# resibots/limbo

Measured on AMD Instinct MI355X. Metric: GP compute()+log_lik evaluations/sec at N=4096 D=6 fp64, higher is better.
Workload: dtype f64

## Files before the change

### limbo_amd/csrc/dev.h

```cpp
#pragma once
#include <hip/hip_runtime.h>
#include <hip/hip_ext.h>
#include <stdint.h>

#define GPE_MAX_THETA 64
#define GPE_MAX_P 8

struct KParams {
    int kind;
    int D;
    int Din;
    int k_lam;
    double sf2;
    double inv_l;
    double diag_add;
    double noise;
    double inv_ell[GPE_MAX_THETA];
};

typedef double d4_t __attribute__((ext_vector_type(4)));

static __device__ __forceinline__ d4_t mfma_f64(double a, double b, d4_t c)
{
    return __builtin_amdgcn_mfma_f64_16x16x4f64(a, b, c, 0, 0, 0);
// ... 117 lines not shown
    double A[GPE_MAX_THETA];
};
void launch_lambda_rows(hipStream_t s, double* Xt, int64_t ld, int64_t col0, int64_t n, const LamParams& lp);

void launch_diag(hipStream_t s, double* A, int64_t lda, int jb, double* Xt, int* info, int64_t goff, int half_form);
typedef unsigned long long gpe_epoch_t;
void launch_panel_step(hipStream_t s, double* A, int64_t lda, int64_t j0, int64_t M, int nt, const double* Xt_cur,
                       double* Xt_next, int do_next, int* info, double* Hs, int64_t dnext, int64_t dfirst, int dinit,
                       double* Dacc, gpe_epoch_t* hflag);
void launch_panel256(hipStream_t s, double* A, int64_t lda, int64_t p0, int64_t M, double* Xt, int* info, int64_t dnext,
                     double* Dacc, double* S22, double* S22_next, hipEvent_t stop = nullptr);
#define GPE_TAIL_MAX 8192
void flow_gate_enter(hipStream_t s);
void flow_gate_leave(hipStream_t s);
void flow_gate_forget(hipStream_t s);
struct FlowGate {
    hipStream_t s;
    bool on;
    explicit FlowGate(hipStream_t s_, bool engage = true) : s(s_), on(engage)
    {
        if (on)
            flow_gate_enter(s);
    }
    ~FlowGate()
    {
        if (on)
            flow_gate_leave(s);
    }
    FlowGate(const FlowGate&) = delete;
    FlowGate& operator=(const FlowGate&) = delete;
};
int debug_tail_order(int nt, int nb, int lag, int pair);
void debug_chain_split(int wave, int* units10, int* cols);
static inline int64_t tail_tiles(int64_t nt, int64_t nb) { return nt * nb - nt * (nt - 1) / 2; }
static inline int64_t tail_buf_doubles(int64_t nt, int64_t nb) { return nt * 3072 + tail_tiles(nt, nb) * 4096; }
struct TailGen {
    const double* Xg;
    int64_t ldx, Ns;
    const double* Om;
    int64_t ldom;
    double* Al;
    int64_t ldal;
    int P;
    const KParams* kp;
};
int ragged_split(int64_t k, int64_t scratch_doubles, int* kc_out);
bool launch_ragged_finish(hipStream_t s, double* C, int64_t ldc, const double* A, int64_t ld, int64_t jb, int64_t P, int64_t k,
                          double* scratch, int64_t scratch_doubles, double* Xt, int* info, int64_t goff);
bool launch_ragged_update(hipStream_t s, double* C, int64_t ldc, const double* A, int64_t ld, int64_t m, int64_t n, int64_t k,
                          double* scratch, int64_t scratch_doubles);
void launch_tail(hipStream_t s, double* A, int64_t lda, int64_t t0, int64_t t1, int64_t N64, int64_t M, double* Xt_all, int* info,
                 double* buf_cur, double* buf_next, const TailGen* gen = nullptr);
#define GPE_S22_TILE 20
#define GPE_S22_TILES 9
#define GPE_HEAD_TILES 66
void launch_head_copy(hipStream_t s, double* A, int64_t lda, int64_t p0, int nt0, int nf, const double* H);
void launch_diag_inv(hipStream_t s, const double* L, int64_t ldl, int64_t N, int64_t b0, int64_t nblocks,
                     double* Xt_all);

struct GemmArgs {
    double* C; int64_t ldc;
    const double* A; int64_t lda; int a_kmajor;
    const double* B; int64_t ldb; int b_kmajor;
    int64_t m, n, k;
    int tri; int64_t grow0, gcol0;
    int ktri;
// ... 149 lines not shown
```

### limbo_amd/csrc/engine.hip

```cpp
#include "../../include/gpe.h"
#include "../../include/gpe_joint.h"
#include "dev.h"

#include <algorithm>
#include <cmath>
#include <cstdio>
#include <cstdlib>
#include <cstring>
#include <iterator>
#include <atomic>
#include <chrono>
#include <map>
#include <dlfcn.h>
#include <fcntl.h>
#include <sys/file.h>
#include <sys/stat.h>
#include <thread>
#include <unistd.h>
#include <mutex>
#include <string>
#include <vector>

thread_local BatchLaunch g_batch;

namespace {
struct TraceRec {
    const char* name;
    hipStream_t stream;
    hipEvent_t e0, e1;
    unsigned gx, gy, gz, bx;
    bool own_stop;
};
std::mutex g_trace_mu;
std::vector<TraceRec> g_trace;
// ... 1525 lines not shown
    std::lock_guard<std::mutex> lk(g_trace_mu);
    for (auto& r : g_trace) {
        g_trace_pool.push_back(r.e0);
        g_trace_pool.push_back(r.e1);
    }
    g_trace.clear();
    g_trace_state.store(on ? 1 : 0);
    return GPE_OK;
}
int gpe_trace_dump(const char* path)
{
    if (!path)
        return GPE_ERR_ARG;
    hipDeviceSynchronize();
    std::lock_guard<std::mutex> lk(g_trace_mu);
    FILE* f = fopen(path, "w");
    if (!f)
        return GPE_ERR_ARG;
    std::map<hipStream_t, int> sid;
    hipEvent_t ref = g_trace.empty() ? nullptr : g_trace[0].e0;
    for (auto& r : g_trace) {
        float a = 0.f, b = 0.f;
        if (hipEventElapsedTime(&a, ref, r.e0) != hipSuccess || hipEventElapsedTime(&b, ref, r.e1) != hipSuccess)
            continue;
        if (!sid.count(r.stream))
            sid[r.stream] = (int)sid.size();
        fprintf(f, "%10.2f %10.2f %d %s grid=%u,%u,%u block=%u\n", 1e3 * a, 1e3 * b, sid[r.stream], r.name, r.gx, r.gy, r.gz, r.bx);
    }
    fclose(f);
    return GPE_OK;
}

int gpe_debug_tail_order(int nt, int nb, int lag, int pair) { return debug_tail_order(nt, nb, lag, pair); }
int gpe_debug_ragged_split(int64_t k, int64_t scratch_doubles, int* kc)
{
    if (!kc)
        return -1;
    *kc = 0;
    return ragged_split(k, scratch_doubles, kc);
}
int gpe_debug_tri_tile_map(int64_t m, int64_t n, int64_t grow0, int64_t gcol0, int* out, int cap)
{
    if (m <= 0 || n <= 0 || !out || cap <= 0 || (m + 127) / 128 >= 65536 || (n + 127) / 128 >= 32768)
        return -1;
    return debug_tri_tile_map(m, n, grow0, gcol0, out, cap);
}
int gpe_debug_chain_split(int wave, int* units10, int* cols)
{
    if (wave < 0 || wave > 7 || !units10 || !cols)
        return -1;
    debug_chain_split(wave, units10, cols);
    return 0;
}
int gpe_debug_inv_plan(int64_t n, int64_t ld, int nbins, int load_pct, int64_t* out, int64_t cap_rows)
{
    return inv2_debug_plan(n, ld, nbins, load_pct, out, cap_rows);
}

int gpe_debug_tail_plan(int64_t n, int p, int g, int64_t tail_max, int64_t tall_max, int64_t batch_tail_max, int64_t* out8)
{
    if (!out8 || n < 1 || p < 1)
        return GPE_ERR_ARG;
    debug_tail_plan(n, p, g, tail_max, tall_max, batch_tail_max, out8);
    return GPE_OK;
}

// ... 18 lines not shown
```

### limbo_amd/csrc/potrf.hip

```cpp
#include "dev.h"
#include <hip/hip_ext.h>
#include <atomic>
#include <cstdio>

#define NB 64
#ifndef DIAG_ABL
#define DIAG_ABL 0
#endif
#ifdef DIAG_TIMING
__device__ long long g_diag_arr[16][8];
__device__ long long g_diag_ts[32];
#ifdef DIAG_NO_STAMPS
#define ARR(G, w) do { } while (0)
#define TS(i) do { } while (0)
#else
#define ARR(G, w) do { if ((threadIdx.x & 63) == 0 && blockIdx.x == 0) g_diag_arr[G][w] = clock64(); } while (0)
#define TS(i) do { if (threadIdx.x == 0) g_diag_ts[i] = clock64(); } while (0)
#endif
#else
#define TS(i) do { } while (0)
#define ARR(G, w) do { } while (0)
#endif
#ifdef DIAG_TIMING
__device__ long long g_panel_ts[64];
// ... 388 lines not shown
        GPE_LAUNCH(k_diag_full, dim3(1, 1, g_batch.G), dim3(256), 0, s, A, lda, jb, Xt, info, goff, g_batch.bt);
}

#define PS 80

template <bool BKM, int KLEN, int RBN, int BS = XS>
static __device__ __forceinline__ void mmk(const double* __restrict__ Aop, int ak0, const double* __restrict__ Bop,
                                           int bk0, int wm, int wn, int lane, double (&acc)[2][RBN])
{
    const int ar = wm + (lane & 15), bc = wn + (lane & 3), kq = lane >> 4;
#pragma unroll
    for (int ks = 0; ks < KLEN; ks += 4) {
        double af[2], bf[RBN];
#pragma unroll
        for (int x = 0; x < 2; ++x)
            af[x] = Aop[(ak0 + ks + kq) * PS + ar + 16 * x];
#pragma unroll
        for (int x = 0; x < RBN; ++x)
            bf[x] = BKM ? Bop[(bc + 4 * x) * BS + bk0 + ks + kq] : Bop[(bk0 + ks + kq) * PS + bc + 4 * x];
#pragma unroll
        for (int n = 0; n < RBN; ++n)
#pragma unroll
            for (int m = 0; m < 2; ++m)
                acc[m][n] = mfma4(af[m], bf[n], acc[m][n]);
    }
}
template <bool BKM>
static __device__ __forceinline__ void mm64(const double* __restrict__ Aop, const double* __restrict__ Bop, int wm, int wn,
                                            int lane, double (&acc)[2][4])
{
    mmk<BKM, NB, 4>(Aop, 0, Bop, 0, wm, wn, lane, acc);
}

static __device__ __forceinline__ void trsm_tile_full(double* __restrict__ T, const double* __restrict__ Bx, int lane, int wave)
{
    const int wm = (wave & 1) * 32, wn = (wave >> 1) * 16;
    const int drow = 4 * ((lane >> 2) & 3) + (lane >> 4), dcol = lane & 3;
    double y[2][4];
#pragma unroll
    for (int m = 0; m < 2; ++m)
#pragma unroll
        for (int n = 0; n < 4; ++n)
            y[m][n] = 0.0;
    switch (wave >> 1) {
    case 0: mmk<true, 16, 4>(T, 0, Bx, 0, wm, wn, lane, y); break;
    case 1: mmk<true, 32, 4>(T, 0, Bx, 0, wm, wn, lane, y); break;
    case 2: mmk<true, 48, 4>(T, 0, Bx, 0, wm, wn, lane, y); break;
    default: mmk<true, 64, 4>(T, 0, Bx, 0, wm, wn, lane, y); break;
    }
    __syncthreads();
#pragma unroll
    for (int m = 0; m < 2; ++m)
#pragma unroll
        for (int n = 0; n < 4; ++n)
            T[(wn + 4 * n + dcol) * PS + wm + 16 * m + drow] = y[m][n];
    __syncthreads();
}

struct TileRegs {
    double v[8];
    __device__ __forceinline__ void load(const double* __restrict__ G, int64_t ld, int nrows)
    {
        const int i = threadIdx.x & 63, kk0 = threadIdx.x >> 6;
        const int ic = i < nrows ? i : nrows - 1;
#pragma unroll
        for (int q = 0; q < 8; ++q)
// ... 333 lines not shown
            b[q] = __hip_atomic_load(g + 8 * q * NB, __ATOMIC_RELAXED, POLL_FIRST_SCOPE);
    }
    __device__ __forceinline__ void finish(const double* G, int spin_limit, int* __restrict__ info)
    {
        const unsigned long long SENT = ~0ull;
        const unsigned long long* g = reinterpret_cast<const unsigned long long*>(G) + (threadIdx.x & 63) + (threadIdx.x >> 6) * NB;
        int spins = 0;
        while (b[0] == SENT || b[1] == SENT || b[2] == SENT || b[3] == SENT || b[4] == SENT || b[5] == SENT || b[6] == SENT
               || b[7] == SENT) {
            if (++spins > spin_limit) {
                info[2] = 1;
                break;
            }
            poll_one(G + NB * NB - 1, spin_limit, info);
            if (b[0] == SENT) b[0] = __hip_atomic_load(g + 0 * NB, __ATOMIC_RELAXED, __HIP_MEMORY_SCOPE_AGENT);
            if (b[1] == SENT) b[1] = __hip_atomic_load(g + 8 * NB, __ATOMIC_RELAXED, __HIP_MEMORY_SCOPE_AGENT);
            if (b[2] == SENT) b[2] = __hip_atomic_load(g + 16 * NB, __ATOMIC_RELAXED, __HIP_MEMORY_SCOPE_AGENT);
            if (b[3] == SENT) b[3] = __hip_atomic_load(g + 24 * NB, __ATOMIC_RELAXED, __HIP_MEMORY_SCOPE_AGENT);
            if (b[4] == SENT) b[4] = __hip_atomic_load(g + 32 * NB, __ATOMIC_RELAXED, __HIP_MEMORY_SCOPE_AGENT);
            if (b[5] == SENT) b[5] = __hip_atomic_load(g + 40 * NB, __ATOMIC_RELAXED, __HIP_MEMORY_SCOPE_AGENT);
            if (b[6] == SENT) b[6] = __hip_atomic_load(g + 48 * NB, __ATOMIC_RELAXED, __HIP_MEMORY_SCOPE_AGENT);
            if (b[7] == SENT) b[7] = __hip_atomic_load(g + 56 * NB, __ATOMIC_RELAXED, __HIP_MEMORY_SCOPE_AGENT);
        }
    }
    __device__ __forceinline__ void store(double* __restrict__ T) const
    {
        const int i = threadIdx.x & 63, kk0 = threadIdx.x >> 6;
#pragma unroll
        for (int q = 0; q < 8; ++q)
            T[(kk0 + 8 * q) * PS + i] = __longlong_as_double((long long)b[q]);
    }
};

template <int S, bool PUBHALF>
static __device__ __forceinline__ void p256_half_solve(const P256& x, double* __restrict__ T, double* __restrict__ Ld,
                                                       const double (&own)[8], double (&a2)[2][4], const bool acc_on,
                                                       const double* __restrict__ Sq, double* __restrict__ pub)
{
    const int lane = threadIdx.x & 63, wave = __builtin_amdgcn_readfirstlane(threadIdx.x >> 6);
    const int wm = (wave & 1) * 32, wn = (wave >> 1) * 16;
    const int hn = (wave >> 1) * 8;
    const int crow = wm + (lane & 31), ccol = wn + (lane >> 5);
    const int drow = 4 * ((lane >> 2) & 3) + (lane >> 4), dcol = lane & 3;
    double* Bx = x.Bx;
    P2TS(6 * S + 0);
#pragma unroll
    for (int it = 0; it < 8; ++it)
        T[(ccol + 2 * it) * PS + crow] = own[it];
    const unsigned long long SENT = ~0ull;
    const unsigned long long* Sp = reinterpret_cast<const unsigned long long*>(Sq) + threadIdx.x;
    {
        unsigned long long b[4];
#pragma unroll
        for (int q = 0; q < 4; ++q)
            b[q] = __hip_atomic_load(Sp + 512 * q, __ATOMIC_RELAXED, POLL_FIRST_SCOPE);
        int spins = 0;
        while (b[0] == SENT || b[1] == SENT || b[2] == SENT || b[3] == SENT) {
            if (++spins > x.spin_limit) {
                x.info[2] = 1;
                break;
            }
            poll_one(Sq + 1023, x.spin_limit, x.info);
            poll_one(Sq + 1024 + 32 * 31, x.spin_limit, x.info);
#pragma unroll
            for (int q = 0; q < 4; ++q)
                if (b[q] == SENT)
// ... 330 lines not shown
    static const bool fault = getenv("GPE_HANDOVER_FAULT") && atoi(getenv("GPE_HANDOVER_FAULT")) != 0;
    const int spin_limit = fault ? -16 : GPE_FLOW_SPIN_LIMIT;
    const int64_t rows = M - (p0 + NB);
    if (rows <= 0)
        return;
    const dim3 grid((unsigned)((rows + NB - 1) / NB)), block(512);
    FlowGate gate(s);
    if (stop)
        GPE_LAUNCH_STOP("k_panel256", k_panel256, grid, block, 0, s, stop, A, lda, p0, M, Xt, info, dnext, Dacc, spin_limit, S22, S22_next);
    else
        GPE_LAUNCH(k_panel256, grid, block, 0, s, A, lda, p0, M, Xt, info, dnext, Dacc, spin_limit, S22, S22_next);
}

struct TailArgs {
    double* A;
    int64_t lda, t0;
    int nt, nb;
    int nfull;
    int rhs_rows;
    double* Xt;
    int* info;
    double *LP, *SP, *LPn, *SPn;
    int spin_limit;
    const int* order;
    const double* Xg;
    int64_t ldx, Ns;
    const double* Om;
    int64_t ldom;
    double* Al;
    int64_t ldal;
    int P;
};
#define TAIL_LDS_DOUBLES (4 * NB * PS)
static_assert(TAIL_LDS_DOUBLES >= NB * XS + 3 * NB * PS && TAIL_LDS_DOUBLES * 8 <= 160 * 1024, "k_tail LDS carve");
static __device__ __forceinline__ int tail_tile_id(int nb, int b, int c) { return c * nb - (c * (c - 1)) / 2 + (b - c); }

static __device__ __forceinline__ void tail_gen_tile(const TailArgs& a, const KParams* __restrict__ kp, int64_t I, int64_t J0,
                                                     double (&out)[8])
{
    if (I >= a.Ns) {
        const double* om = a.Om + (I - a.Ns) * a.ldom;
#pragma unroll
        for (int it = 0; it < 8; ++it)
            out[it] = om[J0 + 2 * it];
        return;
    }
    double z[8];
#pragma unroll
    for (int it = 0; it < 8; ++it)
        z[it] = 0.0;
    const int D = kp->D;
    for (int d = 0; d < D; ++d) {
        const double* xr = a.Xg + (int64_t)d * a.ldx;
        const double xi = xr[I], ie = kp->inv_ell[d];
#pragma unroll
        for (int it = 0; it < 8; ++it) {
            const double q = (xi - xr[J0 + 2 * it]) * ie;
            z[it] = fma(q, q, z[it]);
        }
    }
    const int kind = kp->kind;
    const double sf2 = kp->sf2, da = kp->diag_add;
#pragma unroll
    for (int it = 0; it < 8; ++it)
        out[it] = kfun_fast_rt(kind, z[it], sf2) + (I == J0 + 2 * it ? da : 0.0);
}

// ... 301 lines not shown
        X22[(e0 >> 5) * 34 + (e0 & 31)] = __longlong_as_double((long long)xc[0]);
        X22[(e1 >> 5) * 34 + (e1 & 31)] = __longlong_as_double((long long)xc[1]);
    }
    __syncthreads();
    TTS2(x, true, 3);
    double y2[2][2] = {{0.0, 0.0}, {0.0, 0.0}};
    tri_solve32(T, 32, X22, wm, hn, lane, y2);
#pragma unroll
    for (int m = 0; m < 2; ++m)
#pragma unroll
        for (int n = 0; n < 2; ++n)
            Ys[(hn + 4 * n + dcol) * PS + wm + 16 * m + drow] = y2[m][n];
    __syncthreads();
    TTS2(x, true, 4);
    syrk40<32>(Ys, 0, wave, lane, a2v);
    syrk40_store_neg(Dl, wave, lane, a2v);
    {
        const int i = threadIdx.x & 63, kk0 = threadIdx.x >> 6;
#pragma unroll
        for (int q = 0; q < 4; ++q) {
            const int col = kk0 + 8 * q;
            __hip_atomic_store(pub + i + NB * (32 + col), Ys[col * PS + i], __ATOMIC_RELAXED, __HIP_MEMORY_SCOPE_AGENT);
        }
    }
#pragma unroll
    for (int m = 0; m < 2; ++m)
#pragma unroll
        for (int n = 0; n < 2; ++n)
            T[(32 + hn + 4 * n + dcol) * PS + wm + 16 * m + drow] = y2[m][n];
    TTS2(x, true, 5);
}

static __device__ __forceinline__ void tail_tile_solve(const P256& x, double* __restrict__ lds, const double (&own)[8],
                                                       const double* __restrict__ Sq, double* __restrict__ pub, const bool near)
{
    const int lane = threadIdx.x & 63, wave = __builtin_amdgcn_readfirstlane(threadIdx.x >> 6);
    const int wm = (wave & 1) * 32, wn = (wave >> 1) * 16;
    const int hn = tri_solve_cols(wave);
    const int crow = wm + (lane & 31), ccol = wn + (lane >> 5);
    const int drow = 4 * ((lane >> 2) & 3) + (lane >> 4), dcol = lane & 3;
    double* const T = lds + CH_T;
    double* const X11 = lds + CH_X11;
    double* const Ld = lds + CH_LD;
    double* const Ys = lds + CH_YS;
    double* const X22 = lds + CH_X22;
    const unsigned long long SENT = ~0ull;
    const unsigned long long* Sp = reinterpret_cast<const unsigned long long*>(Sq) + threadIdx.x;
#pragma unroll
    for (int it = 0; it < 8; ++it)
        T[(ccol + 2 * it) * PS + crow] = own[it];
    {
        unsigned long long xb[4];
#pragma unroll
        for (int q = 0; q < 4; ++q)
            xb[q] = __hip_atomic_load(Sp + 512 * q, __ATOMIC_RELAXED, POLL_FIRST_SCOPE);
        if (near)
            chain_watch<4>(Sp, xb, x.spin_limit, x.info);
        else {
            int spins = 0;
            while (xb[0] == SENT || xb[1] == SENT || xb[2] == SENT || xb[3] == SENT) {
                if (++spins > x.spin_limit) {
                    x.info[2] = 1;
                    break;
                }
                poll_one(Sq + 1023, x.spin_limit, x.info);
                poll_one(Sq + 1024 + 32 * 31, x.spin_limit, x.info);
#pragma unroll
                for (int q = 0; q < 4; ++q)
                    if (xb[q] == SENT)
                        xb[q] = __hip_atomic_load(Sp + 512 * q, __ATOMIC_RELAXED, __HIP_MEMORY_SCOPE_AGENT);
            }
        }
#pragma unroll
        for (int q = 0; q < 2; ++q) {
            const int e = threadIdx.x + 512 * q;
            X11[(e >> 5) * 34 + (e & 31)] = __longlong_as_double((long long)xb[q]);
            Ld[(e & 31) * 34 + (e >> 5)] = __longlong_as_double((long long)xb[2 + q]);
        }
    }
    __syncthreads();
    double y1[2][2] = {{0.0, 0.0}, {0.0, 0.0}};
    tri_solve32(T, 0, X11, wm, hn, lane, y1);
#pragma unroll
    for (int m = 0; m < 2; ++m)
#pragma unroll
        for (int n = 0; n < 2; ++n)
            Ys[(hn + 4 * n + dcol) * PS + wm + 16 * m + drow] = y1[m][n];
    __syncthreads();
    double u[2][2] = {{0.0, 0.0}, {0.0, 0.0}};
    mmk<true, 32, 2, 34>(Ys, 0, Ld, 0, wm, hn, lane, u);
#pragma unroll
    for (int m = 0; m < 2; ++m)
#pragma unroll
        for (int n = 0; n < 2; ++n) {
            double* t = T + (32 + hn + 4 * n + dcol) * PS + wm + 16 * m + drow;
            *t = *t - u[m][n];
            T[(hn + 4 * n + dcol) * PS + wm + 16 * m + drow] = y1[m][n];
        }
    {
        const int i = threadIdx.x & 63, kk0 = threadIdx.x >> 6;
#pragma unroll
        for (int q = 0; q < 4; ++q) {
            const int col = kk0 + 8 * q;
            __hip_atomic_store(pub + i + NB * col, Ys[col * PS + i], __ATOMIC_RELAXED, __HIP_MEMORY_SCOPE_AGENT);
        }
    }
    {
        unsigned long long xc[2];
        xc[0] = __hip_atomic_load(Sp + 2048, __ATOMIC_RELAXED, POLL_FIRST_SCOPE);
        xc[1] = __hip_atomic_load(Sp + 2048 + 512, __ATOMIC_RELAXED, POLL_FIRST_SCOPE);
        if (near)
            chain_watch<2>(Sp + 2048, xc, x.spin_limit, x.info);
        else {
            int spins = 0;
            while (xc[0] == SENT || xc[1] == SENT) {
                if (++spins > x.spin_limit) {
                    x.info[2] = 1;
                    break;
                }
                poll_one(Sq + 2048 + 1023, x.spin_limit, x.info);
                if (xc[0] == SENT)
                    xc[0] = __hip_atomic_load(Sp + 2048, __ATOMIC_RELAXED, __HIP_MEMORY_SCOPE_AGENT);
                if (xc[1] == SENT)
                    xc[1] = __hip_atomic_load(Sp + 2048 + 512, __ATOMIC_RELAXED, __HIP_MEMORY_SCOPE_AGENT);
            }
        }
        const int e0 = threadIdx.x, e1 = threadIdx.x + 512;
        X22[(e0 >> 5) * 34 + (e0 & 31)] = __longlong_as_double((long long)xc[0]);
        X22[(e1 >> 5) * 34 + (e1 & 31)] = __longlong_as_double((long long)xc[1]);
    }
    __syncthreads();
    double y2[2][2] = {{0.0, 0.0}, {0.0, 0.0}};
    tri_solve32(T, 32, X22, wm, hn, lane, y2);
#pragma unroll
    for (int m = 0; m < 2; ++m)
#pragma unroll
        for (int n = 0; n < 2; ++n)
            Ys[(hn + 4 * n + dcol) * PS + wm + 16 * m + drow] = y2[m][n];
    __syncthreads();
    {
        const int i = threadIdx.x & 63, kk0 = threadIdx.x >> 6;
#pragma unroll
        for (int q = 0; q < 4; ++q) {
            const int col = kk0 + 8 * q;
            __hip_atomic_store(pub + i + NB * (32 + col), Ys[col * PS + i], __ATOMIC_RELAXED, __HIP_MEMORY_SCOPE_AGENT);
        }
    }
#pragma unroll
    for (int m = 0; m < 2; ++m)
#pragma unroll
        for (int n = 0; n < 2; ++n)
            T[(32 + hn + 4 * n + dcol) * PS + wm + 16 * m + drow] = y2[m][n];
    __syncthreads();
}

static __device__ __forceinline__ void tail_body(const TailArgs& a, const int wgid, double* __restrict__ lds,
                                                 const KParams* __restrict__ kp = nullptr)
{
    const int lane = threadIdx.x & 63, wave = __builtin_amdgcn_readfirstlane(threadIdx.x >> 6);
    const int wm = (wave & 1) * 32, wn = (wave >> 1) * 16;
    const int crow = wm + (lane & 31), ccol = wn + (lane >> 5);
    int c = 0, b;
    if (a.order) {
        b = __builtin_amdgcn_readfirstlane(a.order[2 * wgid]);
        c = __builtin_amdgcn_readfirstlane(a.order[2 * wgid + 1]);
    }
    else {
        int id = wgid, colh = a.nb;
        while (id >= colh) {
            id -= colh;
            ++c;
            --colh;
        }
        b = c + id;
    }
    const int slot = tail_tile_id(a.nb, b, c);
    const bool mute = a.spin_limit < 0;
    P256 x;
    x.A = a.A;
    x.lda = a.lda;
    x.p0 = a.t0;
    x.R0 = a.t0 + (int64_t)NB * b;
    x.Xt = a.Xt;
    x.info = a.info;
    x.mute = mute;
    x.spin_limit = mute ? -a.spin_limit : a.spin_limit;
    x.nrows = b < a.nfull ? NB : a.rhs_rows;
    x.want_d = false;
    x.Bx = lds;
    x.T0 = lds + NB * XS;
    x.T1 = x.T0 + NB * PS;
    x.T2 = x.T1 + NB * PS;
    x.S22 = a.SP;
    x.HP = a.LP;
    double* const myslot = a.LP + (int64_t)slot * (NB * NB);
    {
        unsigned long long* nx = reinterpret_cast<unsigned long long*>(a.LPn + (int64_t)slot * (NB * NB));
#pragma unroll
        for (int q = 0; q < 8; ++q)
            nx[threadIdx.x + 512 * q] = ~0ull;
        if (b == c) {
            unsigned long long* ns = reinterpret_cast<unsigned long long*>(a.SPn + (int64_t)c * 3072);
#pragma unroll
            for (int q = 0; q < 6; ++q)
                ns[threadIdx.x + 512 * q] = ~0ull;
        }
    }
    if (b == c + 1 && b < a.nt)
        return;
    const int crc = crow < x.nrows ? crow : x.nrows - 1;
    double cv[8];
    if (kp) {
        tail_gen_tile(a, kp, x.R0 + crc, a.t0 + (int64_t)NB * c + ccol, cv);
        if (a.Al && b >= a.nfull && threadIdx.x < NB)
            for (int p = 0; p < a.P; ++p)
                reinterpret_cast<unsigned long long*>(a.Al)[a.t0 + (int64_t)NB * c + threadIdx.x + (int64_t)p * a.ldal] = ~0ull;
    }
    else {
#pragma unroll
        for (int it = 0; it < 8; ++it)
            cv[it] = a.A[x.R0 + crc + (a.t0 + (int64_t)NB * c + ccol + 2 * it) * a.lda];
    }
    if (b == c) {
        double* const Dl = lds + CH_D;
        double* const Ltb = lds + CH_AUX;
        double* const invd = Ltb + DIAG_LTB;
        DiagSync* const sy = reinterpret_cast<DiagSync*>(invd + NB);
        if (c > 0) {
            double cl[8];
            if (kp)
                tail_gen_tile(a, kp, x.R0 + crow, a.t0 + (int64_t)NB * (c - 1) + ccol, cl);
            else {
#pragma unroll
                for (int it = 0; it < 8; ++it)
                    cl[it] = a.A[x.R0 + crow + (a.t0 + (int64_t)NB * (c - 1) + ccol + 2 * it) * a.lda];
            }
            tail_chain_updates_and_crossing(a, x, lds, c, cl, cv);
            TTS(c, 1);
        }
        else {
#pragma unroll
            for (int it = 0; it < 8; ++it)
                Dl[crow * XS + ccol + 2 * it] = cv[it];
            diag_flow_init(sy);
        }
        __syncthreads();
        DiagEarly ea;
        ea.mute = mute;
        ea.S = a.SP + (int64_t)c * 3072;
        TTS(c, 2);
        diag_flow(Dl, Ltb, invd, sy, a.A + x.R0 + x.R0 * a.lda, a.lda, a.Xt + (int64_t)c * (NB * NB), a.info, x.R0, wave, lane,
                  invd + NB + 8, &ea);
        TTS(c, 3);
        if (c > 0) {
            __syncthreads();
            const int i = threadIdx.x & 63, kk0 = threadIdx.x >> 6;
            double* Ag = a.A + x.R0 + (a.t0 + (int64_t)NB * (c - 1)) * a.lda;
            const double* T = lds + CH_T;
#pragma unroll
            for (int q = 0; q < 8; ++q) {
                const int col = kk0 + 8 * q;
                Ag[i + (int64_t)col * a.lda] = T[col * PS + i];
            }
        }
        return;
    }
    PolledTile pa, pb;
    if (c > 0) {
        pa.issue(a.LP + (int64_t)tail_tile_id(a.nb, b, 0) * (NB * NB));
        pb.issue(a.LP + (int64_t)tail_tile_id(a.nb, c, 0) * (NB * NB));
    }
    double a2[2][4] = {{0.0, 0.0, 0.0, 0.0}, {0.0, 0.0, 0.0, 0.0}};
#pragma unroll 1
    for (int s = 0; s < c; ++s) {
        double* const opA = lds + (s & 1) * (2 * NB * PS);
        double* const opB = opA + NB * PS;
        pa.finish(a.LP + (int64_t)tail_tile_id(a.nb, b, s) * (NB * NB), x.spin_limit, x.info);
        pa.store(opA);
        pb.finish(a.LP + (int64_t)tail_tile_id(a.nb, c, s) * (NB * NB), x.spin_limit, x.info);
        pb.store(opB);
        if (s + 1 < c) {
            pa.issue(a.LP + (int64_t)tail_tile_id(a.nb, b, s + 1) * (NB * NB));
            pb.issue(a.LP + (int64_t)tail_tile_id(a.nb, c, s + 1) * (NB * NB));
        }
        __syncthreads();
        mm64<false>(opA, opB, wm, wn, lane, a2);
    }
    if (c > 0) {
        double a2r[8];
        wave_tile_to_rows(a2, a2r, lane);
#pragma unroll
        for (int it = 0; it < 8; ++it)
            cv[it] -= a2r[it];
        __syncthreads();
    }
    tail_tile_solve(x, lds, cv, a.SP + (int64_t)c * 3072, myslot, b - c <= 3);
    {
// ... 264 lines not shown
        const int me = pos[tid(t.b, t.c)];
        if (t.b == t.c) {
            int last = -1;
            for (int s2 = 0; s2 < t.c - 1; ++s2)
                last = std::max(last, std::max(owner(t.c, s2), owner(t.c - 1, s2)));
            if (last > me) {
                if (dlead <= 0)
                    legal = false;
                ++blocked[(size_t)me + 1];
                --blocked[(size_t)last + 1];
            }
            if (t.c > 0)
                legal = legal && dpos(t.c - 1) < me;
        }
        else if (!(t.b == t.c + 1 && t.b < nt)) {
            for (int s2 = 0; s2 < t.c && legal; ++s2)
                legal = owner(t.b, s2) < me && owner(t.c, s2) < me;
            legal = legal && dpos(t.c) < me;
        }
        if (!legal)
            break;
    }
    for (size_t q = 1, run = 0; q < blocked.size() && legal; ++q) {
        run += blocked[q];
        legal = (int)run <= TAIL_DLEAD_MAX_BLOCKED;
    }
    flat.assign(2 * ts.size(), 0);
    for (size_t i = 0; i < ts.size(); ++i) {
        flat[2 * i] = ts[i].b;
        flat[2 * i + 1] = ts[i].c;
    }
    return legal;
}
static const int* tail_order(int nt, int nb, int dlead, int lag)
{
    const int W = 0;
    if (dlead <= 0 && lag <= 0)
        return nullptr;
    static std::mutex mu;
    static std::map<std::array<int, 6>, int*> cache;
    int dev = 0;
    (void)hipGetDevice(&dev);
    const std::array<int, 6> key{dev, nt, nb, dlead, lag, 0};
    std::lock_guard<std::mutex> lk(mu);
    auto it = cache.find(key);
    if (it != cache.end())
        return it->second;
    std::vector<int> flat;
    int* d = nullptr;
    if (build_tail_order(nt, nb, W, lag, flat, dlead) || (dlead > 0 && build_tail_order(nt, nb, W, lag, flat, 0))) {
        if (hipMalloc(&d, sizeof(int) * flat.size()) != hipSuccess || hipMemcpy(d, flat.data(), sizeof(int) * flat.size(), hipMemcpyHostToDevice) != hipSuccess)
            d = nullptr;
    }
    else
        fprintf(stderr, "gpe: tail_order(%d, %d, lead %d, lag %d) violates a dependency — column-by-column order used\n", nt, nb, dlead, lag);
    cache[key] = d;
    return d;
}
void debug_chain_split(int wave, int* units10, int* cols)
{
    for (int q = 0; q < 5; ++q)
        syrk40_units(wave, q, units10[2 * q], units10[2 * q + 1]);
    *cols = tri_solve_cols(wave);
}
int debug_tail_order(int nt, int nb, int lag, int pair)
{
    if (pair)
        return -1;
    if (nt < 1 || nb < nt || nb > 4096)
        return -1;
    std::vector<int> flat;
    if (!build_tail_order(nt, nb, 0, lag, flat, 0))
        return 0;
    if (!build_tail_order(nt, nb, 0, lag, flat, TAIL_DLEAD))
        return 0;
    std::vector<char> seen((size_t)nt * nb, 0);
    size_t n = 0;
    for (size_t i = 0; i + 1 < flat.size(); i += 2) {
        const int b = flat[i], c = flat[i + 1];
        if (c < 0 || c >= nt || b < c || b >= nb || seen[(size_t)c * nb + b])
            return 0;
        seen[(size_t)c * nb + b] = 1;
        ++n;
    }
    return n == (size_t)(nt * nb - nt * (nt - 1) / 2) ? 1 : 0;
}

void launch_tail(hipStream_t s, double* A, int64_t lda, int64_t t0, int64_t t1, int64_t N64, int64_t M, double* Xt_all, int* info,
                 double* buf_cur, double* buf_next, const TailGen* gen)
{
    TailArgs a{};
    a.A = A;
    a.lda = lda;
    a.t0 = t0;
    a.nt = (int)((t1 - t0) / NB);
    a.nfull = (int)((N64 - t0) / NB);
    a.rhs_rows = (int)(M - N64);
    a.nb = a.nfull + (a.rhs_rows > 0 ? 1 : 0);
    a.Xt = Xt_all + (t0 / NB) * (NB * NB);
    a.info = info;
    a.SP = buf_cur;
    a.LP = buf_cur + (int64_t)a.nt * 3072;
    a.SPn = buf_next;
    a.LPn = buf_next + (int64_t)a.nt * 3072;
    static const bool fault = getenv("GPE_HANDOVER_FAULT") && atoi(getenv("GPE_HANDOVER_FAULT")) != 0;
    a.spin_limit = fault ? -16 : GPE_FLOW_SPIN_LIMIT;
    static const int ord_lag = getenv("GPE_TAIL_LAG") ? atoi(getenv("GPE_TAIL_LAG")) : 3;
    a.order = tail_order(a.nt, a.nb, g_batch.bt ? 0 : TAIL_DLEAD, ord_lag);
    const int64_t tiles = tail_tiles(a.nt, a.nb);
    if (gen) {
        a.Xg = gen->Xg;
        a.ldx = gen->ldx;
        a.Ns = gen->Ns;
        a.Om = gen->Om;
        a.ldom = gen->ldom;
        a.Al = gen->Al;
        a.ldal = gen->ldal;
        a.P = gen->P;
    }
    FlowGate gate(s);
    if (g_batch.bt)
        GPE_LAUNCH(k_tail_b, dim3((unsigned)(tiles * g_batch.G)), dim3(512), 0, s, a, g_batch.bt);
    else if (gen)
        GPE_LAUNCH(k_tail_g, dim3((unsigned)tiles), dim3(512), 0, s, a, *gen->kp);
    else
        GPE_LAUNCH(k_tail, dim3((unsigned)tiles), dim3(512), 0, s, a);
}

__global__ __launch_bounds__(512) void k_upd_fused(GemmArgs g, double* __restrict__ A, int64_t lda, int64_t p0, int64_t pe,
                                                   double* __restrict__ Xt_next, int* __restrict__ info,
                                                   const double* __restrict__ Dacc)
{
    constexpr int GEMM_LDS = 4 * Glds64Shape<16>::STAGE, DIAG_LDS = 2 * NB * PS;
    constexpr int LDS_DOUBLES = GEMM_LDS > DIAG_LDS ? GEMM_LDS : DIAG_LDS;
    __shared__ __attribute__((aligned(16))) double lds[LDS_DOUBLES];
    if (blockIdx.x + 1 < gridDim.x) {
        gemm_glds64_body<16, 4, 8>(g, lds, (int)blockIdx.x, (int)gridDim.x - 1, true);
        return;
    }
    static_assert(NB * XS + DIAG_LTB + NB + 8 + DIAG_XW_DOUBLES <= 2 * NB * PS,
                  "[Ls | Ltb | invd | sync | Xw] is carved out of the two operand tiles");
    double* T0 = lds;
// ... 214 lines not shown
```

Measured before the change: 939.5.

## Pair vertically adjacent tail tiles in one workgroup to share B operand loads

Adds a 'duo' mode to the Cholesky tail kernel. One workgroup now updates and solves two vertically adjacent off-diagonal tiles of the same column, reusing the shared B-panel and the triangular factor fetch across both. A new dependency-checked ordering builder emits paired entries flagged by a high bit, and the launch grid shrinks to the number of entries. This cuts global polling and loads and the workgroup count, at the cost of longer per-workgroup critical paths, more LDS use and less parallelism in the dependency-driven schedule.

```diff
diff --git a/include/gpe_tail_duo.h b/include/gpe_tail_duo.h
--- /dev/null
+++ b/include/gpe_tail_duo.h
@@ -0,0 +1,17 @@
+#ifndef GPE_TAIL_DUO_H
+#define GPE_TAIL_DUO_H
+
+#include "gpe.h"
+
+#ifdef __cplusplus
+extern "C" {
+#endif
+
+#define GPE_TAIL_DUO_BIT 0x40000000
+
+int gpe_debug_tail_duo_order(int nt, int nb, int nfull, int lag, int strict, int* out, int cap);
+
+#ifdef __cplusplus
+}
+#endif
+#endif
diff --git a/limbo_amd/csrc/dev.h b/limbo_amd/csrc/dev.h
--- a/limbo_amd/csrc/dev.h
+++ b/limbo_amd/csrc/dev.h
@@ -173,6 +173,7 @@
 };
 int debug_tail_order(int nt, int nb, int lag, int pair);
 void debug_chain_split(int wave, int* units10, int* cols);
+int debug_tail_duo_order(int nt, int nb, int nfull, int lag, int strict, int* out, int cap);
 static inline int64_t tail_tiles(int64_t nt, int64_t nb) { return nt * nb - nt * (nt - 1) / 2; }
 static inline int64_t tail_buf_doubles(int64_t nt, int64_t nb) { return nt * 3072 + tail_tiles(nt, nb) * 4096; }
 struct TailGen {
diff --git a/limbo_amd/csrc/engine.hip b/limbo_amd/csrc/engine.hip
--- a/limbo_amd/csrc/engine.hip
+++ b/limbo_amd/csrc/engine.hip
@@ -1,5 +1,6 @@
 #include "../../include/gpe.h"
 #include "../../include/gpe_joint.h"
+#include "../../include/gpe_tail_duo.h"
 #include "dev.h"
 
 #include <algorithm>
@@ -1591,6 +1592,10 @@
 }
 
 int gpe_debug_tail_order(int nt, int nb, int lag, int pair) { return debug_tail_order(nt, nb, lag, pair); }
+int gpe_debug_tail_duo_order(int nt, int nb, int nfull, int lag, int strict, int* out, int cap)
+{
+    return debug_tail_duo_order(nt, nb, nfull, lag, strict, out, cap);
+}
 int gpe_debug_ragged_split(int64_t k, int64_t scratch_doubles, int* kc)
 {
     if (!kc)
diff --git a/limbo_amd/csrc/potrf.hip b/limbo_amd/csrc/potrf.hip
--- a/limbo_amd/csrc/potrf.hip
+++ b/limbo_amd/csrc/potrf.hip
@@ -444,6 +444,32 @@
     mmk<BKM, NB, 4>(Aop, 0, Bop, 0, wm, wn, lane, acc);
 }
 
+template <int KLEN>
+static __device__ __forceinline__ void mmk2(const double* __restrict__ A0, const double* __restrict__ A1, const double* __restrict__ Bop,
+                                            int wm, int wn, int lane, double (&acc0)[2][4], double (&acc1)[2][4])
+{
+    const int ar = wm + (lane & 15), bc = wn + (lane & 3), kq = lane >> 4;
+#pragma unroll
+    for (int ks = 0; ks < KLEN; ks += 4) {
+        double af0[2], af1[2], bf[4];
+#pragma unroll
+        for (int x = 0; x < 2; ++x) {
+            af0[x] = A0[(ks + kq) * PS + ar + 16 * x];
+            af1[x] = A1[(ks + kq) * PS + ar + 16 * x];
+        }
+#pragma unroll
+        for (int x = 0; x < 4; ++x)
+            bf[x] = Bop[(ks + kq) * PS + bc + 4 * x];
+#pragma unroll
+        for (int n = 0; n < 4; ++n)
+#pragma unroll
+            for (int m = 0; m < 2; ++m) {
+                acc0[m][n] = mfma4(af0[m], bf[n], acc0[m][n]);
+                acc1[m][n] = mfma4(af1[m], bf[n], acc1[m][n]);
+            }
+    }
+}
+
 static __device__ __forceinline__ void trsm_tile_full(double* __restrict__ T, const double* __restrict__ Bx, int lane, int wave)
 {
     const int wm = (wave & 1) * 32, wn = (wave >> 1) * 16;
@@ -843,6 +869,41 @@
     }
 };
 
+struct PolledHalf {
+    unsigned long long b[4];
+    __device__ __forceinline__ void issue(const double* G, int H)
+    {
+        const unsigned long long* g = reinterpret_cast<const unsigned long long*>(G) + (threadIdx.x & 63) + ((threadIdx.x >> 6) + 32 * H) * NB;
+#pragma unroll
+        for (int q = 0; q < 4; ++q)
+            b[q] = __hip_atomic_load(g + 8 * q * NB, __ATOMIC_RELAXED, POLL_FIRST_SCOPE);
+    }
+    __device__ __forceinline__ void finish(const double* G, int H, int spin_limit, int* __restrict__ info)
+    {
+        const unsigned long long SENT = ~0ull;
+        const unsigned long long* g = reinterpret_cast<const unsigned long long*>(G) + (threadIdx.x & 63) + ((threadIdx.x >> 6) + 32 * H) * NB;
+        int spins = 0;
+        while (b[0] == SENT || b[1] == SENT || b[2] == SENT || b[3] == SENT) {
+            if (++spins > spin_limit) {
+                info[2] = 1;
+                break;
+            }
+            poll_one(G + 32 * NB * (H + 1) - 1, spin_limit, info);
+            if (b[0] == SENT) b[0] = __hip_atomic_load(g + 0 * NB, __ATOMIC_RELAXED, __HIP_MEMORY_SCOPE_AGENT);
+            if (b[1] == SENT) b[1] = __hip_atomic_load(g + 8 * NB, __ATOMIC_RELAXED, __HIP_MEMORY_SCOPE_AGENT);
+            if (b[2] == SENT) b[2] = __hip_atomic_load(g + 16 * NB, __ATOMIC_RELAXED, __HIP_MEMORY_SCOPE_AGENT);
+            if (b[3] == SENT) b[3] = __hip_atomic_load(g + 24 * NB, __ATOMIC_RELAXED, __HIP_MEMORY_SCOPE_AGENT);
+        }
+    }
+    __device__ __forceinline__ void store(double* __restrict__ T) const
+    {
+        const int i = threadIdx.x & 63, kk0 = threadIdx.x >> 6;
+#pragma unroll
+        for (int q = 0; q < 4; ++q)
+            T[(kk0 + 8 * q) * PS + i] = __longlong_as_double((long long)b[q]);
+    }
+};
+
 template <int S, bool PUBHALF>
 static __device__ __forceinline__ void p256_half_solve(const P256& x, double* __restrict__ T, double* __restrict__ Ld,
                                                        const double (&own)[8], double (&a2)[2][4], const bool acc_on,
@@ -1239,7 +1300,9 @@
     int P;
 };
 #define TAIL_LDS_DOUBLES (4 * NB * PS)
+#define TAIL_DUO_BIT (1 << 30)
 static_assert(TAIL_LDS_DOUBLES >= NB * XS + 3 * NB * PS && TAIL_LDS_DOUBLES * 8 <= 160 * 1024, "k_tail LDS carve");
+static_assert(6 * 32 * PS <= TAIL_LDS_DOUBLES, "k_tail LDS carve of a pair workgroup: two sets of three k-half operands");
 static __device__ __forceinline__ int tail_tile_id(int nb, int b, int c) { return c * nb - (c * (c - 1)) / 2 + (b - c); }
 
 static __device__ __forceinline__ void tail_gen_tile(const TailArgs& a, const KParams* __restrict__ kp, int64_t I, int64_t J0,
@@ -1607,7 +1670,8 @@
 }
 
 static __device__ __forceinline__ void tail_tile_solve(const P256& x, double* __restrict__ lds, const double (&own)[8],
-                                                       const double* __restrict__ Sq, double* __restrict__ pub, const bool near)
+                                                       const double* __restrict__ Sq, double* __restrict__ pub, const bool near,
+                                                       const bool fetch = true)
 {
     const int lane = threadIdx.x & 63, wave = __builtin_amdgcn_readfirstlane(threadIdx.x >> 6);
     const int wm = (wave & 1) * 32, wn = (wave >> 1) * 16;
@@ -1624,7 +1688,7 @@
 #pragma unroll
     for (int it = 0; it < 8; ++it)
         T[(ccol + 2 * it) * PS + crow] = own[it];
-    {
+    if (fetch) {
         unsigned long long xb[4];
 #pragma unroll
         for (int q = 0; q < 4; ++q)
@@ -1680,7 +1744,7 @@
             __hip_atomic_store(pub + i + NB * col, Ys[col * PS + i], __ATOMIC_RELAXED, __HIP_MEMORY_SCOPE_AGENT);
         }
     }
-    {
+    if (fetch) {
         unsigned long long xc[2];
         xc[0] = __hip_atomic_load(Sp + 2048, __ATOMIC_RELAXED, POLL_FIRST_SCOPE);
         xc[1] = __hip_atomic_load(Sp + 2048 + 512, __ATOMIC_RELAXED, POLL_FIRST_SCOPE);
@@ -1729,6 +1793,96 @@
     __syncthreads();
 }
 
+static __device__ __forceinline__ void tail_pair(const TailArgs& a, const P256& x, double* __restrict__ lds, const int b, const int c,
+                                                 double (&cv)[8], double* __restrict__ myslot, const KParams* __restrict__ kp)
+{
+    const int lane = threadIdx.x & 63, wave = __builtin_amdgcn_readfirstlane(threadIdx.x >> 6);
+    const int wm = (wave & 1) * 32, wn = (wave >> 1) * 16;
+    const int crow = wm + (lane & 31), ccol = wn + (lane >> 5);
+    P256 x1 = x;
+    x1.R0 = x.R0 + NB;
+    double cu[8];
+    if (kp)
+        tail_gen_tile(a, kp, x1.R0 + crow, a.t0 + (int64_t)NB * c + ccol, cu);
+    else {
+#pragma unroll
+        for (int it = 0; it < 8; ++it)
+            cu[it] = a.A[x1.R0 + crow + (a.t0 + (int64_t)NB * c + ccol + 2 * it) * a.lda];
+    }
+    if (c > 0) {
+        PolledHalf pa, pu, pb;
+        {
+            const double* Ga = a.LP + (int64_t)tail_tile_id(a.nb, b, 0) * (NB * NB);
+            pa.issue(Ga, 0);
+            pu.issue(Ga + NB * NB, 0);
+            pb.issue(a.LP + (int64_t)tail_tile_id(a.nb, c, 0) * (NB * NB), 0);
+        }
+        double a2[2][4] = {{0.0, 0.0, 0.0, 0.0}, {0.0, 0.0, 0.0, 0.0}};
+        double a3[2][4] = {{0.0, 0.0, 0.0, 0.0}, {0.0, 0.0, 0.0, 0.0}};
+#pragma unroll 1
+        for (int s = 0; s < c; ++s) {
+            const double* Ga = a.LP + (int64_t)tail_tile_id(a.nb, b, s) * (NB * NB);
+            const double* Gb = a.LP + (int64_t)tail_tile_id(a.nb, c, s) * (NB * NB);
+#pragma unroll
+            for (int H = 0; H < 2; ++H) {
+                double* const opA = lds + H * (3 * 32 * PS);
+                double* const opU = opA + 32 * PS;
+                double* const opB = opU + 32 * PS;
+                pa.finish(Ga, H, x.spin_limit, x.info);
+                pa.store(opA);
+                pu.finish(Ga + NB * NB, H, x.spin_limit, x.info);
+                pu.store(opU);
+                pb.finish(Gb, H, x.spin_limit, x.info);
+                pb.store(opB);
+                if (H == 0) {
+                    pa.issue(Ga, 1);
+                    pu.issue(Ga + NB * NB, 1);
+                    pb.issue(Gb, 1);
+                }
+                else if (s + 1 < c) {
+                    const double* Gn = a.LP + (int64_t)tail_tile_id(a.nb, b, s + 1) * (NB * NB);
+                    pa.issue(Gn, 0);
+                    pu.issue(Gn + NB * NB, 0);
+                    pb.issue(a.LP + (int64_t)tail_tile_id(a.nb, c, s + 1) * (NB * NB), 0);
+                }
+                __syncthreads();
+                mmk2<32>(opA, opU, opB, wm, wn, lane, a2, a3);
+            }
+        }
+        double r[8];
+        wave_tile_to_rows(a2, r, lane);
+#pragma unroll
+        for (int it = 0; it < 8; ++it)
+            cv[it] -= r[it];
+        wave_tile_to_rows(a3, r, lane);
+#pragma unroll
+        for (int it = 0; it < 8; ++it)
+            cu[it] -= r[it];
+        __syncthreads();
+    }
+    const int i = threadIdx.x & 63, kk0 = threadIdx.x >> 6;
+    const double* T = lds + CH_T;
+    tail_tile_solve(x, lds, cv, a.SP + (int64_t)c * 3072, myslot, false);
+    {
+        double* Ag = a.A + x.R0 + (a.t0 + (int64_t)NB * c) * a.lda;
+#pragma unroll
+        for (int q = 0; q < 8; ++q) {
+            const int col = kk0 + 8 * q;
+            Ag[i + (int64_t)col * a.lda] = T[col * PS + i];
+        }
+    }
+    __syncthreads();
+    tail_tile_solve(x1, lds, cu, a.SP + (int64_t)c * 3072, myslot + NB * NB, false, false);
+    {
+        double* Ag = a.A + x1.R0 + (a.t0 + (int64_t)NB * c) * a.lda;
+#pragma unroll
+        for (int q = 0; q < 8; ++q) {
+            const int col = kk0 + 8 * q;
+            Ag[i + (int64_t)col * a.lda] = T[col * PS + i];
+        }
+    }
+}
+
 static __device__ __forceinline__ void tail_body(const TailArgs& a, const int wgid, double* __restrict__ lds,
                                                  const KParams* __restrict__ kp = nullptr)
 {
@@ -1736,9 +1890,12 @@
     const int wm = (wave & 1) * 32, wn = (wave >> 1) * 16;
     const int crow = wm + (lane & 31), ccol = wn + (lane >> 5);
     int c = 0, b;
+    bool duo = false;
     if (a.order) {
         b = __builtin_amdgcn_readfirstlane(a.order[2 * wgid]);
         c = __builtin_amdgcn_readfirstlane(a.order[2 * wgid + 1]);
+        duo = (b & TAIL_DUO_BIT) != 0;
+        b &= ~TAIL_DUO_BIT;
     }
     else {
         int id = wgid, colh = a.nb;
@@ -1774,6 +1931,11 @@
 #pragma unroll
         for (int q = 0; q < 8; ++q)
             nx[threadIdx.x + 512 * q] = ~0ull;
+        if (duo) {
+#pragma unroll
+            for (int q = 8; q < 16; ++q)
+                nx[threadIdx.x + 512 * q] = ~0ull;
+        }
         if (b == c) {
             unsigned long long* ns = reinterpret_cast<unsigned long long*>(a.SPn + (int64_t)c * 3072);
 #pragma unroll
@@ -1838,6 +2000,10 @@
                 Ag[i + (int64_t)col * a.lda] = T[col * PS + i];
             }
         }
+        return;
+    }
+    if (duo) {
+        tail_pair(a, x, lds, b, c, cv, myslot, kp);
         return;
     }
     PolledTile pa, pb;
@@ -2168,30 +2334,142 @@
     }
     return legal;
 }
-static const int* tail_order(int nt, int nb, int dlead, int lag)
+static bool build_tail_duo_order(int nt, int nb, int nfull, int lag, std::vector<int>& flat, int dlead)
+{
+    struct T {
+        int key, c, b, duo;
+    };
+    std::vector<T> ts;
+    for (int c = 0; c < nt; ++c)
+        for (int b = c; b < nb; ++b) {
+            int k;
+            if (b == c)
+                k = 2 * c - 3 - 2 * dlead;
+            else if (b >= nt)
+                k = 2 * (c + std::max(lag, 0));
+            else if (b == c + 1)
+                k = 2 * c;
+            else
+                k = 2 * c;
+            const bool duo = b - c >= 4 && b + 1 < nfull && b + 1 < nb && ((b + 1 < nt) || (b >= nt));
+            ts.push_back(T{k, c, b, duo ? 1 : 0});
+            if (duo)
+                ++b;
+        }
+    std::stable_sort(ts.begin(), ts.end(), [](const T& x, const T& y) {
+        if (x.key != y.key)
+            return x.key < y.key;
+        if (x.c != y.c)
+            return x.c < y.c;
+        return x.b < y.b;
+    });
+    auto tid = [&](int b, int c) { return c * nb - (c * (c - 1)) / 2 + (b - c); };
+    std::vector<int> pos((size_t)(nt * nb - nt * (nt - 1) / 2), -1);
+    for (size_t i = 0; i < ts.size(); ++i) {
+        pos[tid(ts[i].b, ts[i].c)] = (int)i;
+        if (ts[i].duo)
+            pos[tid(ts[i].b + 1, ts[i].c)] = (int)i;
+    }
+    auto dpos = [&](int c) { return pos[tid(c, c)]; };
+    auto owner = [&](int b, int s) { return (b == s + 1 && b < nt) ? dpos(b) : pos[tid(b, s)]; };
+    bool legal = true;
+    for (int p : pos)
+        legal = legal && p >= 0;
+    std::vector<int> blocked(ts.size() + 1, 0);
+    for (size_t e = 0; e < ts.size() && legal; ++e) {
+        const T& t = ts[e];
+        const int me = (int)e;
+        if (t.b == t.c) {
+            int last = -1;
+            for (int s2 = 0; s2 < t.c - 1; ++s2)
+                last = std::max(last, std::max(owner(t.c, s2), owner(t.c - 1, s2)));
+            if (last > me) {
+                if (dlead <= 0)
+                    legal = false;
+                ++blocked[(size_t)me + 1];
+                --blocked[(size_t)last + 1];
+            }
+            if (t.c > 0)
+                legal = legal && dpos(t.c - 1) < me;
+        }
+        else if (!(t.b == t.c + 1 && t.b < nt)) {
+            for (int r = t.b; r <= t.b + t.duo; ++r)
+                for (int s2 = 0; s2 < t.c && legal; ++s2)
+                    legal = owner(r, s2) < me && owner(t.c, s2) < me;
+            legal = legal && dpos(t.c) < me;
+        }
+    }
+    for (size_t q = 1, run = 0; q < blocked.size() && legal; ++q) {
+        run += blocked[q];
+        legal = (int)run <= TAIL_DLEAD_MAX_BLOCKED;
+    }
+    flat.assign(2 * ts.size(), 0);
+    for (size_t i = 0; i < ts.size(); ++i) {
+        flat[2 * i] = ts[i].b | (ts[i].duo ? TAIL_DUO_BIT : 0);
+        flat[2 * i + 1] = ts[i].c;
+    }
+    return legal;
+}
+static bool tail_table(int nt, int nb, int nfull, int dlead, int lag, bool duo, std::vector<int>& flat)
 {
     const int W = 0;
-    if (dlead <= 0 && lag <= 0)
+    if (duo && build_tail_duo_order(nt, nb, nfull, lag, flat, dlead))
+        return true;
+    return build_tail_order(nt, nb, W, lag, flat, dlead) || (dlead > 0 && build_tail_order(nt, nb, W, lag, flat, 0));
+}
+static bool tail_duo_on()
+{
+    static const bool on = !getenv("GPE_TAIL_DUO") || atoi(getenv("GPE_TAIL_DUO")) != 0;
+    return on;
+}
+static const int* tail_order(int nt, int nb, int nfull, int dlead, int lag, bool duo, int64_t* entries)
+{
+    *entries = tail_tiles(nt, nb);
+    if (dlead <= 0 && lag <= 0 && !duo)
         return nullptr;
+    struct Tab {
+        int* d;
+        int64_t n;
+    };
     static std::mutex mu;
-    static std::map<std::array<int, 6>, int*> cache;
+    static std::map<std::array<int, 7>, Tab> cache;
     int dev = 0;
     (void)hipGetDevice(&dev);
-    const std::array<int, 6> key{dev, nt, nb, dlead, lag, 0};
+    const std::array<int, 7> key{dev, nt, nb, nfull, dlead, lag, duo ? 1 : 0};
     std::lock_guard<std::mutex> lk(mu);
     auto it = cache.find(key);
-    if (it != cache.end())
-        return it->second;
+    if (it == cache.end()) {
+        std::vector<int> flat;
+        Tab t{nullptr, tail_tiles(nt, nb)};
+        bool ok = tail_table(nt, nb, nfull, dlead, lag, duo, flat);
+        if (!ok)
+            fprintf(stderr, "gpe: tail_order(%d, %d, lead %d, lag %d) violates a dependency — column-by-column order used\n", nt, nb, dlead, lag);
+        for (int pass = 0; ok && pass < 2 && !t.d; ++pass) {
+            if (hipMalloc(&t.d, sizeof(int) * flat.size()) == hipSuccess
+                && hipMemcpy(t.d, flat.data(), sizeof(int) * flat.size(), hipMemcpyHostToDevice) == hipSuccess) {
+                t.n = (int64_t)(flat.size() / 2);
+                break;
+            }
+            if (t.d)
+                (void)hipFree(t.d);
+            t.d = nullptr;
+            ok = duo && pass == 0 && (dlead > 0 || lag > 0) && tail_table(nt, nb, nfull, dlead, lag, false, flat);
+        }
+        it = cache.emplace(key, t).first;
+    }
+    *entries = it->second.n;
+    return it->second.d;
+}
+int debug_tail_duo_order(int nt, int nb, int nfull, int lag, int strict, int* out, int cap)
+{
+    if (nt < 1 || nb < nt || nb > 4096 || nfull < nt || nfull > nb || nfull < nb - 1 || lag < 0 || (cap > 0 && !out))
+        return -1;
     std::vector<int> flat;
-    int* d = nullptr;
-    if (build_tail_order(nt, nb, W, lag, flat, dlead) || (dlead > 0 && build_tail_order(nt, nb, W, lag, flat, 0))) {
-        if (hipMalloc(&d, sizeof(int) * flat.size()) != hipSuccess || hipMemcpy(d, flat.data(), sizeof(int) * flat.size(), hipMemcpyHostToDevice) != hipSuccess)
-            d = nullptr;
-    }
-    else
-        fprintf(stderr, "gpe: tail_order(%d, %d, lead %d, lag %d) violates a dependency — column-by-column order used\n", nt, nb, dlead, lag);
-    cache[key] = d;
-    return d;
+    if (!tail_table(nt, nb, nfull, strict ? 0 : TAIL_DLEAD, lag, true, flat))
+        return -1;
+    for (size_t i = 0; i < flat.size() && (int)i < cap; ++i)
+        out[i] = flat[i];
+    return (int)(flat.size() / 2);
 }
 void debug_chain_split(int wave, int* units10, int* cols)
 {
@@ -2242,8 +2520,8 @@
     static const bool fault = getenv("GPE_HANDOVER_FAULT") && atoi(getenv("GPE_HANDOVER_FAULT")) != 0;
     a.spin_limit = fault ? -16 : GPE_FLOW_SPIN_LIMIT;
     static const int ord_lag = getenv("GPE_TAIL_LAG") ? atoi(getenv("GPE_TAIL_LAG")) : 3;
-    a.order = tail_order(a.nt, a.nb, g_batch.bt ? 0 : TAIL_DLEAD, ord_lag);
-    const int64_t tiles = tail_tiles(a.nt, a.nb);
+    int64_t tiles = 0;
+    a.order = tail_order(a.nt, a.nb, a.nfull, g_batch.bt ? 0 : TAIL_DLEAD, ord_lag, !g_batch.bt && tail_duo_on(), &tiles);
     if (gen) {
         a.Xg = gen->Xg;
         a.ldx = gen->ldx;
```

Result: slower. 777.8 (-17.2%).
